# jinbeizame007/pytorch-r2d2-DPG

Hardware: NVIDIA H100
Metric: learner sequence-steps/sec (batch x seq_len) (higher is better)
Workload: dtype bf16x3 (fp32 operands split into bf16 hi+lo, three tensor-core passes, fp32 accumulate: ~16-bit operands)

## Files before the change

include/r2d2_b200.h:

```cpp
#ifndef R2D2_B200_H_
#define R2D2_B200_H_

#include <stddef.h>
#include <stdint.h>

#ifdef __cplusplus
extern "C" {
#endif

#define R2D2_OK 0
#define R2D2_ERR_CUDA (-1)
#define R2D2_ERR_ARG (-2)
#define R2D2_ERR_UNSUPPORTED (-3)
#define R2D2_ERR_STATE (-4)

typedef void* r2d2_stream_t;

int r2d2_version(void);
const char* r2d2_arch(void);
const char* r2d2_last_error(void);
int r2d2_device_sm_count(int* out);

int r2d2_gemm_f32(int layout, int M, int N, int K, const float* A, long long lda, const float* B, long long ldb,
                  const float* A2, long long lda2, const float* B2, long long ldb2, int K2, float* C,
                  long long ldc, const float* bias, const float* Z, long long ldz, int epilogue, int split_k,
                  r2d2_stream_t stream);

typedef struct {
  int obs_size;
  int n_actions;
  int hidden;
  int is_critic;
} r2d2_net_shape;

size_t r2d2_net_param_count(const r2d2_net_shape* shape);
size_t r2d2_net_workspace_floats(const r2d2_net_shape* shape, int T, int B, int repeat);

int r2d2_lstm_net_forward(const r2d2_net_shape* shape, const float* params, const float* obs, const float* act,
                          const float* h0, const float* c0, int T, int B, int repeat, int head_first_row,
                          float* out, float* workspace, r2d2_stream_t stream);

int r2d2_lstm_net_backward(const r2d2_net_shape* shape, const float* params, const float* obs, const float* act,
                           const float* d_out, int T, int B, int repeat, int head_first_row, float* grads,
                           float* d_act, float* workspace, r2d2_stream_t stream);

int r2d2_lstm_scan_forward(const float* gin, const float* whh, const float* h0, const float* c0, float* gates,
                           float* hs, float* cs, float* head_in, int T, int B, int H, int repeat, float* scratch,
                           r2d2_stream_t stream);
int r2d2_lstm_scan_backward(const float* gates, const float* hs, const float* cs, const float* whh,
                            const float* dh_head, int head_first_step, float* dgates, float* dgin, int T, int B,
                            int H, int repeat, float* scratch, r2d2_stream_t stream);

int r2d2_set_gemm_impl(int impl);
int r2d2_get_gemm_impl(void);
int r2d2_set_scan_impl(int impl);
int r2d2_get_scan_impl(void);
int r2d2_scan_status(int* status, r2d2_stream_t stream);

int r2d2_td_priority(const float* q, const float* q_next, const float* rew, const float* term, int L, int B,
                     int A, int burn_in, int n_step, float gamma, float eta, float* target, float* dq,
                     float* td_sq, float* priority, float* critic_loss, r2d2_stream_t stream);
int r2d2_td_priority_weighted(const float* q, const float* q_next, const float* rew, const float* term,
                              const float* is_weight, int L, int B, int A, int burn_in, int n_step, float gamma, float eta,
                              float* target, float* dq, float* td_sq, float* priority, float* critic_loss,
                              r2d2_stream_t stream);

#define R2D2_RESCALE_REFERENCE 0
#define R2D2_RESCALE_INVERTIBLE 1
#define R2D2_PRIORITY_SQUARED 0
#define R2D2_PRIORITY_ABS 1
typedef struct {
  int rescaling;
  float eps;
  int priority_metric;
} r2d2_td_options;
int r2d2_td_priority_ex(const float* q, const float* q_next, const float* rew, const float* term, const float* is_weight,
                        int L, int B, int A, int burn_in, int n_step, float gamma, float eta, float* target, float* dq,
                        float* td_sq, float* priority, float* critic_loss, const r2d2_td_options* options,
                        r2d2_stream_t stream);

int r2d2_nstep_rewards(const float* raw, const int* n_rows, int T, int B, int n_step, float gamma, float* out,
                       r2d2_stream_t stream);
int r2d2_actor_priorities(const float* q, const float* q_next, const float* rew, const float* term, const int* n_rows,
                          int B, int A, int burn_in, int learning, int n_step, float gamma, float eta, int p_max,
                          float* prio, r2d2_stream_t stream);
int r2d2_actor_priorities_ex(const float* q, const float* q_next, const float* rew, const float* term, const int* n_rows,
                             int B, int A, int burn_in, int learning, int n_step, float gamma, float eta, int p_max,
                             float* prio, const r2d2_td_options* options, r2d2_stream_t stream);

size_t r2d2_policy_workspace_floats(const r2d2_net_shape* shape, int N);
int r2d2_policy_step(const r2d2_net_shape* shape, const float* const params[4], const float* obs,
                     const float* state_in, float* state_out, float* mu, int N, float* workspace,
                     r2d2_stream_t stream);

int r2d2_adam_step(float* params, const float* grads, float* exp_avg, float* exp_avg_sq, long long n, int step,
                   float lr, float beta1, float beta2, float eps, float grad_scale, r2d2_stream_t stream);

typedef struct r2d2_replay r2d2_replay_t;

typedef struct {
  int obs_size, n_actions, hidden;
// ... 105 lines not shown
```

pytorch-r2d2-dpg_b200/csrc/api.cu:

```cuda
#include <atomic>
#include <cmath>

#include "common.cuh"
#include "elementwise.cuh"
#include "gemm.cuh"
#include "learner.cuh"
#include "lstm_scan.cuh"
#include "net.cuh"
#include "policy.cuh"
#include "replay.cuh"

namespace r2d2 {
static thread_local std::string g_last_error;
static std::atomic<long long> g_launches{0};
void set_last_error(const std::string& msg) { g_last_error = msg; }
const char* last_error() { return g_last_error.c_str(); }
void count_launch(int n) { g_launches.fetch_add(n, std::memory_order_relaxed); }
long long launch_count() { return g_launches.load(std::memory_order_relaxed); }
int num_sms() {
  static std::atomic<int> cache[64];
  int dev = 0;
  if (cudaGetDevice(&dev) != cudaSuccess || dev < 0 || dev >= 64) return 132;
  int n = cache[dev].load(std::memory_order_relaxed);
  if (n == 0) {
// ... 39 lines not shown

size_t r2d2_net_param_count(const r2d2_net_shape* shape) { return shape ? shape_of(shape).param_count() : 0; }

size_t r2d2_net_workspace_floats(const r2d2_net_shape* shape, int T, int B, int repeat) {
  return shape ? ChainWs::floats(shape_of(shape), T, B, repeat) : 0;
}

int r2d2_lstm_net_forward(const r2d2_net_shape* shape, const float* params, const float* obs, const float* act,
                          const float* h0, const float* c0, int T, int B, int repeat, int head_first_row,
                          float* out, float* workspace, r2d2_stream_t stream) {
  R2D2_REQUIRE(shape && params && obs && workspace, "null");
  R2D2_REQUIRE(T > 0 && B > 0 && repeat >= 1, "shape");
  const NetShape s = shape_of(shape);
  const NetParams P = NetParams::from_flat(const_cast<float*>(params), s);
  const ChainWs ws = ChainWs::carve(workspace, s, T, B, repeat);
  R2D2_TRY(net_forward(s, P, ws, obs, act, h0, c0, T, B, repeat, S(stream)));
  if (out) {
    float* ho = ws.head_out + (size_t)head_first_row * B * s.act;
    R2D2_TRY(net_head_forward(s, P, ws, head_first_row, T, B, repeat, ho, s.act, S(stream)));
    R2D2_CUDA_TRY(cudaMemcpyAsync(out, ho, sizeof(float) * (size_t)(T - head_first_row) * B * s.act,
                                  cudaMemcpyDeviceToDevice, S(stream)));
  }
  return R2D2_OK;
}

int r2d2_lstm_net_backward(const r2d2_net_shape* shape, const float* params, const float* obs, const float* act,
                           const float* d_out, int T, int B, int repeat, int head_first_row, float* grads,
                           float* d_act, float* workspace, r2d2_stream_t stream) {
  R2D2_REQUIRE(shape && params && obs && d_out && workspace, "null");
  const NetShape s = shape_of(shape);
  const NetParams P = NetParams::from_flat(const_cast<float*>(params), s);
  const ChainWs ws = ChainWs::carve(workspace, s, T, B, repeat);
  const long long n = (long long)(T - head_first_row) * B * s.act;
  const float* d_pre = d_out;
  if (!s.critic) {
    R2D2_TRY(mul_dtanh(d_out, ws.head_out + (size_t)head_first_row * B * s.act, ws.d_pre, n, S(stream)));
    d_pre = ws.d_pre;
  }
  NetParams G;
  if (grads) G = NetParams::from_flat(grads, s);
  return net_backward(s, P, grads ? &G : nullptr, ws, obs, act, d_pre, head_first_row, T, B, repeat, d_act, nullptr,
                      S(stream));
}

int r2d2_lstm_scan_forward(const float* gin, const float* whh, const float* h0, const float* c0, float* gates,
                           float* hs, float* cs, float* head_in, int T, int B, int H, int repeat, float* scratch,
                           r2d2_stream_t stream) {
  ScanFwdParams p;
  p.gin = gin; p.whh = whh; p.h0 = h0; p.c0 = c0; p.gates = gates; p.hs = hs; p.cs = cs; p.head_in = head_in;
  p.T = T; p.B = B; p.H = H; p.repeat = repeat; p.scratch = scratch;
  return lstm_scan_forward(p, S(stream));
}

int r2d2_lstm_scan_backward(const float* gates, const float* hs, const float* cs, const float* whh,
                            const float* dh_head, int head_first_step, float* dgates, float* dgin, int T, int B,
                            int H, int repeat, float* scratch, r2d2_stream_t stream) {
  ScanBwdParams p;
  p.gates = gates; p.hs = hs; p.cs = cs; p.whh = whh; p.dh_head = dh_head; p.head_first_step = head_first_step;
  p.dgates = dgates; p.dgin = dgin; p.T = T; p.B = B; p.H = H; p.repeat = repeat; p.scratch = scratch;
  return lstm_scan_backward(p, S(stream));
}

int r2d2_set_gemm_impl(int impl) {
  gemm_set_impl(impl != 0);
  gemm_set_impl_skinny_mma(impl != 2);
  return R2D2_OK;
}
int r2d2_get_gemm_impl(void) { return gemm_get_impl(); }
int r2d2_set_scan_impl(int impl) { lstm_scan_set_impl(impl); return R2D2_OK; }
int r2d2_get_scan_impl(void) { return lstm_scan_get_impl(); }
int r2d2_scan_status(int* status, r2d2_stream_t stream) { return lstm_scan_error_status(status, S(stream)); }

int r2d2_td_priority(const float* q, const float* q_next, const float* rew, const float* term, int L, int B,
                     int A, int burn_in, int n_step, float gamma, float eta, float* target, float* dq,
                     float* td_sq, float* priority, float* critic_loss, r2d2_stream_t stream) {
  TdPriorityParams p;
  p.q = q; p.q_next = q_next; p.rew = rew; p.term = term; p.target = target; p.dq = dq; p.td_sq = td_sq;
  p.priority = priority; p.loss_sum = critic_loss; p.L = L; p.B = B; p.A = A; p.burn_in = burn_in; p.n_step = n_step;
  p.gamma_n = (float)pow((double)gamma, (double)n_step);
  p.eta = eta;
  return td_priority(p, S(stream));
}

int r2d2_td_priority_weighted(const float* q, const float* q_next, const float* rew, const float* term,
                              const float* is_weight, int L, int B, int A, int burn_in, int n_step, float gamma, float eta,
                              float* target, float* dq, float* td_sq, float* priority, float* critic_loss,
                              r2d2_stream_t stream) {
  TdPriorityParams p;
  p.q = q; p.q_next = q_next; p.rew = rew; p.term = term; p.target = target; p.dq = dq; p.td_sq = td_sq;
  p.priority = priority; p.loss_sum = critic_loss; p.L = L; p.B = B; p.A = A; p.burn_in = burn_in; p.n_step = n_step;
  p.gamma_n = (float)pow((double)gamma, (double)n_step);
  p.eta = eta;
  p.is_weight = is_weight;
  return td_priority(p, S(stream));
}

static int td_options_of(const r2d2_td_options* o, TdOptions* out) {
  *out = TdOptions();
  if (o) { out->rescaling = o->rescaling; out->eps = o->eps; out->priority_metric = o->priority_metric; }
  return check_td_options(*out);
}

int r2d2_td_priority_ex(const float* q, const float* q_next, const float* rew, const float* term, const float* is_weight,
                        int L, int B, int A, int burn_in, int n_step, float gamma, float eta, float* target, float* dq,
                        float* td_sq, float* priority, float* critic_loss, const r2d2_td_options* options,
                        r2d2_stream_t stream) {
// ... 243 lines not shown
```

pytorch-r2d2-dpg_b200/csrc/lstm_scan.cu:

```cuda
#include <cooperative_groups.h>
#include <stdlib.h>

#include "gemm.cuh"
#include "lstm_scan.cuh"
#include "elementwise.cuh"
#include "sm90.cuh"

namespace cg = cooperative_groups;

namespace r2d2 {
namespace {

constexpr int SCAN_THREADS = 256;
constexpr int UNITS_PER_CTA = 32;
constexpr int ROWS_PER_CTA = 128;
constexpr int GT_LD = ROWS_PER_CTA + 4;
constexpr int DG_LD = ROWS_PER_CTA + 8;
constexpr unsigned long long kWaitLimitNs = 4000000000ull;

__device__ unsigned g_scan_status = 0;

__device__ __forceinline__ float accurate_sigmoid(float x) { return 1.0f / (1.0f + expf(-x)); }

__device__ __forceinline__ unsigned long long global_ns() {
  unsigned long long t;
  asm volatile("mov.u64 %0, %globaltimer;" : "=l"(t));
  return t;
}

__device__ __forceinline__ void wait_slice(uint64_t* bar, uint32_t parity) {
  if (sm90::mbar_try_wait(bar, parity)) return;
  if (*reinterpret_cast<volatile unsigned*>(&g_scan_status)) return;
  const unsigned long long t0 = global_ns();
  while (!sm90::mbar_try_wait(bar, parity)) {
    if (global_ns() - t0 > kWaitLimitNs) {
      atomicExch(&g_scan_status, 1u);
      return;
    }
  }
}

__device__ __forceinline__ uint32_t slice_parity(int s) { return (uint32_t)((s - 1) >> 1) & 1u; }

template <int H> __host__ __device__ constexpr bool w_hi_in_smem() { return H > 256; }

template <int H, int NB>
struct FwdSmem {
  static constexpr int C = H / 32;
  static constexpr int HROW = UNITS_PER_CTA + 8;
  static constexpr int SLICE = 2 * NB * HROW;
  static constexpr int W_BYTES = w_hi_in_smem<H>() ? (H / 16) * 8 * 32 * 16 : 0;
  static constexpr int HB_ELEMS = 2 * C * SLICE;
  static constexpr int GT_ELEMS = NB * GT_LD;
  static constexpr int HS_ELEMS = SLICE;
  static constexpr int BAR_OFF = W_BYTES + HB_ELEMS * 2 + GT_ELEMS * 4 + HS_ELEMS * 2;
  static constexpr int BYTES = BAR_OFF + 2 * C * 8;
  static_assert((SLICE * 2) % 16 == 0 && BAR_OFF % 16 == 0, "bulk copies need 16-byte granules");
  static_assert(BYTES <= 232448, "forward scan tile does not fit in 227 KB of shared memory");
};

template <int H, int NB>
__global__ void __launch_bounds__(SCAN_THREADS, 1) lstm_scan_fwd_kernel(ScanFwdParams p) {
  constexpr int C = H / 32, KS = H / 16, NT = NB / 8;
  constexpr bool WS = w_hi_in_smem<H>();
  using SM = FwdSmem<H, NB>;
  constexpr int HROW = SM::HROW, SLICE = SM::SLICE;
  cg::cluster_group cluster = cg::this_cluster();
  const int rank = (int)cluster.block_rank();
  const int b0 = (blockIdx.x / C) * NB;
  const int tid = threadIdx.x, lane = tid & 31, w = tid >> 5;
  const int g = lane >> 2, c = lane & 3;
  const int B = p.B, S = p.T * p.repeat;

  extern __shared__ __align__(16) unsigned char smem_raw[];
  uint4* w_hi_s = reinterpret_cast<uint4*>(smem_raw);
  __nv_bfloat16* hb = reinterpret_cast<__nv_bfloat16*>(smem_raw + SM::W_BYTES);
  float* gt = reinterpret_cast<float*>(smem_raw + SM::W_BYTES + SM::HB_ELEMS * 2);
  __nv_bfloat16* hstage = reinterpret_cast<__nv_bfloat16*>(smem_raw + SM::W_BYTES + SM::HB_ELEMS * 2 + SM::GT_ELEMS * 4);
  uint64_t* bar = reinterpret_cast<uint64_t*>(smem_raw + SM::BAR_OFF);

  for (int idx = tid; idx < NB * H; idx += SCAN_THREADS) {
    const int n = idx / H, k = idx % H, b = b0 + n;
    float v = (b < B && p.h0) ? __ldg(p.h0 + (size_t)b * H + k) : 0.f;
    __nv_bfloat16 hi, lo;
    split_bf16(v, hi, lo);
    __nv_bfloat16* row = hb + (0 * C + k / UNITS_PER_CTA) * SLICE + n * HROW + k % UNITS_PER_CTA;
    row[0] = hi;
    row[NB * HROW] = lo;
  }
  const int ug = rank * 32 + lane;
  float cst[NT];
#pragma unroll
  for (int e = 0; e < NT; ++e) {
    const int b = b0 + w + 8 * e;
    cst[e] = 0.f;
    if (b < B) {
      float hv = p.h0 ? __ldg(p.h0 + (size_t)b * H + ug) : 0.f;
      float cv = p.c0 ? __ldg(p.c0 + (size_t)b * H + ug) : 0.f;
      p.hs[(size_t)b * H + ug] = hv;
      p.cs[(size_t)b * H + ug] = cv;
      cst[e] = cv;
    }
  }
  if (tid < 2 * C) {
    sm90::mbar_init(bar + tid, 1);
    sm90::fence_mbar_init_cluster();
    sm90::mbar_arrive_expect_tx(bar + tid, SLICE * 2);
  }

  uint32_t a_hi[WS ? 1 : KS][4], a_lo[KS][4];
  {
    const int gate = w >> 1;
    const int u_lo = (w & 1) * 16 + g;
    const float* w_r0 = p.whh + (size_t)(gate * H + rank * 32 + u_lo) * H;
    const float* w_r1 = w_r0 + (size_t)8 * H;
#pragma unroll
    for (int ks = 0; ks < KS; ++ks) {
      const int k = ks * 16 + 2 * c;
      float2 v0 = __ldg(reinterpret_cast<const float2*>(w_r0 + k));
      float2 v1 = __ldg(reinterpret_cast<const float2*>(w_r1 + k));
      float2 v2 = __ldg(reinterpret_cast<const float2*>(w_r0 + k + 8));
      float2 v3 = __ldg(reinterpret_cast<const float2*>(w_r1 + k + 8));
      uint32_t h[4];
      split_pack2(v0.x, v0.y, h[0], a_lo[ks][0]);
      split_pack2(v1.x, v1.y, h[1], a_lo[ks][1]);
      split_pack2(v2.x, v2.y, h[2], a_lo[ks][2]);
      split_pack2(v3.x, v3.y, h[3], a_lo[ks][3]);
      if constexpr (WS) {
        w_hi_s[(ks * 8 + w) * 32 + lane] = make_uint4(h[0], h[1], h[2], h[3]);
      } else {
#pragma unroll
        for (int f = 0; f < 4; ++f) a_hi[ks][f] = h[f];
      }
    }
  }
  __syncthreads();
  cluster.sync();

  const size_t gstride = (size_t)4 * H;
  for (int s = 0; s < S; ++s) {
    const int cur = s & 1, nxt = cur ^ 1;
    const int t = s / p.repeat;

#pragma unroll
    for (int nt = 0; nt < NT; ++nt)
#pragma unroll
      for (int f = 0; f < 4; ++f) {
        const int n = nt * 8 + 2 * c + (f & 1), r = 16 * w + g + (f >> 1) * 8, b = b0 + n;
        if (b < B) sm90::cp_async_4(gt + n * GT_LD + r, p.gin + ((size_t)t * B + b) * gstride + (r >> 5) * H + rank * 32 + (r & 31));
      }
    sm90::cp_async_commit();

    float acc[NT][4];
#pragma unroll
    for (int nt = 0; nt < NT; ++nt)
#pragma unroll
      for (int e = 0; e < 4; ++e) acc[nt][e] = 0.f;
    const __nv_bfloat16* hb_cur = hb + cur * C * SLICE;
    uint64_t* bar_cur = bar + cur * C;
    const uint32_t parity = slice_parity(s);
#pragma unroll
    for (int ks = 0; ks < KS; ++ks) {
      if ((ks & 1) == 0 && s > 0) wait_slice(bar_cur + ks / 2, parity);
      const __nv_bfloat16* hb_hi = hb_cur + (ks / 2) * SLICE;
      const __nv_bfloat16* hb_lo = hb_hi + NB * HROW;
      uint32_t ah[4];
      if constexpr (WS) {
        const uint4 v = w_hi_s[(ks * 8 + w) * 32 + lane];
        ah[0] = v.x; ah[1] = v.y; ah[2] = v.z; ah[3] = v.w;
      } else {
#pragma unroll
        for (int f = 0; f < 4; ++f) ah[f] = a_hi[ks][f];
      }
#pragma unroll
      for (int nt = 0; nt < NT; ++nt) {
        const int off = (nt * 8 + g) * HROW + (ks & 1) * 16 + 2 * c;
        uint32_t bh[2], bl[2];
        bh[0] = *reinterpret_cast<const uint32_t*>(hb_hi + off);
        bh[1] = *reinterpret_cast<const uint32_t*>(hb_hi + off + 8);
        bl[0] = *reinterpret_cast<const uint32_t*>(hb_lo + off);
        bl[1] = *reinterpret_cast<const uint32_t*>(hb_lo + off + 8);
        mma_bf16_16816(acc[nt], a_lo[ks], bh);
        mma_bf16_16816(acc[nt], ah, bl);
        mma_bf16_16816(acc[nt], ah, bh);
      }
    }
    sm90::cp_async_wait_all();
#pragma unroll
    for (int nt = 0; nt < NT; ++nt) {
      const int n = nt * 8 + 2 * c, r = 16 * w + g;
      gt[n * GT_LD + r] += acc[nt][0];
      gt[(n + 1) * GT_LD + r] += acc[nt][1];
      gt[n * GT_LD + r + 8] += acc[nt][2];
      gt[(n + 1) * GT_LD + r + 8] += acc[nt][3];
    }
    if (w == 0 && lane < C) sm90::bulk_wait_read_all();
    __syncthreads();
    if (s > 0 && tid < C) sm90::mbar_arrive_expect_tx(bar_cur + tid, SLICE * 2);

#pragma unroll
    for (int e = 0; e < NT; ++e) {
      const int n = w + 8 * e, b = b0 + n;
      __nv_bfloat16 hi = __float2bfloat16_rn(0.f), lo = hi;
      if (b < B) {
        const float* gr = gt + n * GT_LD + lane;
        const float ig = accurate_sigmoid(gr[0]);
        const float fg = accurate_sigmoid(gr[32]);
        const float gg = tanhf(gr[64]);
        const float og = accurate_sigmoid(gr[96]);
        const float cn = fg * cst[e] + ig * gg;
        const float hn = og * tanhf(cn);
        cst[e] = cn;
        if (!p.no_save) {
          float* go = p.gates + ((size_t)s * B + b) * gstride + ug;
          go[0] = ig; go[H] = fg; go[2 * H] = gg; go[3 * H] = og;
          p.cs[((size_t)(s + 1) * B + b) * H + ug] = cn;
        }
        p.hs[((size_t)(s + 1) * B + b) * H + ug] = hn;
        if (p.head_in && (s % p.repeat) == p.repeat - 1)
          p.head_in[((size_t)t * B + b) * H + ug] = tanhf(hn);
        split_bf16(hn, hi, lo);
      }
      hstage[(0 * NB + n) * HROW + lane] = hi;
      hstage[(1 * NB + n) * HROW + lane] = lo;
    }
    sm90::fence_proxy_async_smem();
    __syncthreads();

    if (s + 1 < S && w == 0 && lane < C) {
      const uint32_t slot = sm90::smem_u32(hb + (nxt * C + rank) * SLICE);
      const uint32_t slot_bar = sm90::smem_u32(bar + nxt * C + rank);
      sm90::bulk_copy_s2cluster(sm90::map_cluster(slot, lane), sm90::smem_u32(hstage), SLICE * 2,
                                sm90::map_cluster(slot_bar, lane));
      sm90::bulk_commit();
    }
  }
  cluster.sync();
}

template <int H, int NB>
struct BwdSmem {
  static constexpr int C = H / 32;
  static constexpr int DG_ELEMS = 2 * NB * DG_LD;
  static constexpr int PS_LD = NB + 2;
  static constexpr int PS_ELEMS = 2 * C * UNITS_PER_CTA * PS_LD;
  static constexpr int PS_BYTES_PER_SRC = UNITS_PER_CTA * NB * 4;
  static constexpr int MT = (H / 16 + 7) / 8;
  static constexpr int W_BYTES = w_hi_in_smem<H>() ? MT * 8 * 8 * 32 * 16 : 0;
  static constexpr int STAGE_PLANES = 6;
  static constexpr int STAGE_ELEMS = STAGE_PLANES * NB * UNITS_PER_CTA;
  static constexpr int BAR_OFF = W_BYTES + DG_ELEMS * 2 + PS_ELEMS * 4 + STAGE_ELEMS * 4;
  static constexpr int BYTES = BAR_OFF + 2 * C * 8;
  static_assert(BAR_OFF % 8 == 0, "mbarrier alignment");
  static_assert(BYTES <= 232448, "BPTT scan tile does not fit in 227 KB of shared memory");
};

template <int H, int NB>
__global__ void __launch_bounds__(SCAN_THREADS, 1) lstm_scan_bwd_kernel(ScanBwdParams p) {
  constexpr int C = H / 32, NT = NB / 8;
  constexpr int M_TILES = H / 16;
  constexpr int MT = (M_TILES + 7) / 8;
  constexpr int KS = ROWS_PER_CTA / 16;
  constexpr bool WS = w_hi_in_smem<H>();
  using SM = BwdSmem<H, NB>;
  cg::cluster_group cluster = cg::this_cluster();
  const int rank = (int)cluster.block_rank();
  const int b0 = (blockIdx.x / C) * NB;
  const int tid = threadIdx.x, lane = tid & 31, w = tid >> 5;
  const int g = lane >> 2, c = lane & 3;
  const int B = p.B, S = p.T * p.repeat;

  extern __shared__ __align__(16) unsigned char smem_raw[];
  uint4* w_hi_s = reinterpret_cast<uint4*>(smem_raw);
  __nv_bfloat16* dgs = reinterpret_cast<__nv_bfloat16*>(smem_raw + SM::W_BYTES);
  float* ps = reinterpret_cast<float*>(smem_raw + SM::W_BYTES + SM::DG_ELEMS * 2);
  float* stage = ps + SM::PS_ELEMS;
  uint64_t* bar = reinterpret_cast<uint64_t*>(smem_raw + SM::BAR_OFF);
  constexpr int PLANE = NB * UNITS_PER_CTA;
  constexpr size_t gstride = (size_t)4 * H;

  auto head_step = [&](int s) {
    const int rel = s - p.head_first_step;
// ... 307 lines not shown
int set_cluster_attributes(Kern kern, int cluster_size, int smem_bytes) {
  R2D2_CUDA_TRY(cudaFuncSetAttribute(kern, cudaFuncAttributeMaxDynamicSharedMemorySize, smem_bytes));
  if (cluster_size > 8) R2D2_CUDA_TRY(cudaFuncSetAttribute(kern, cudaFuncAttributeNonPortableClusterSizeAllowed, 1));
  return R2D2_OK;
}

cudaLaunchConfig_t cluster_config(int cluster_size, int n_clusters, int smem_bytes, cudaStream_t stream,
                                  cudaLaunchAttribute* attr) {
  cudaLaunchConfig_t cfg = {};
  cfg.gridDim = dim3(cluster_size * n_clusters);
  cfg.blockDim = dim3(SCAN_THREADS);
  cfg.dynamicSmemBytes = smem_bytes;
  cfg.stream = stream;
  attr[0].id = cudaLaunchAttributeClusterDimension;
  attr[0].val.clusterDim.x = cluster_size;
  attr[0].val.clusterDim.y = 1;
  attr[0].val.clusterDim.z = 1;
  cfg.attrs = attr;
  cfg.numAttrs = 1;
  return cfg;
}

template <typename Kern, typename Params>
int launch_cluster(Kern kern, const Params& p, int cluster_size, int n_clusters, int smem_bytes, cudaStream_t stream) {
  R2D2_TRY(set_cluster_attributes(kern, cluster_size, smem_bytes));
  cudaLaunchAttribute attr[1];
  cudaLaunchConfig_t cfg = cluster_config(cluster_size, n_clusters, smem_bytes, stream, attr);
  R2D2_CUDA_TRY(cudaLaunchKernelEx(&cfg, kern, p));
  count_launch();
  return R2D2_OK;
}

template <typename Kern>
int resident_clusters(Kern kern, int cluster_size, int smem_bytes, int* out) {
  R2D2_TRY(set_cluster_attributes(kern, cluster_size, smem_bytes));
  cudaLaunchAttribute attr[1];
  cudaLaunchConfig_t cfg = cluster_config(cluster_size, 1, smem_bytes, nullptr, attr);
  R2D2_CUDA_TRY(cudaOccupancyMaxActiveClusters(out, kern, &cfg));
  return R2D2_OK;
}

template <int H, typename K8, typename K16, typename K32>
int pick_nb(int B, K8 k8, int smem8, K16 k16, int smem16, K32 k32, int smem32, int* nb) {
  int fit = 0;
  R2D2_TRY(resident_clusters(k8, H / 32, smem8, &fit));
  if (ceil_div(B, 8) <= fit) { *nb = 8; return R2D2_OK; }
  R2D2_TRY(resident_clusters(k16, H / 32, smem16, &fit));
  if (ceil_div(B, 16) <= fit || !k32) { *nb = 16; return R2D2_OK; }
  *nb = 32;
  (void)smem32;
  return R2D2_OK;
}

template <int H>
int fwd_dispatch(const ScanFwdParams& p, cudaStream_t stream) {
  constexpr bool WIDE = !w_hi_in_smem<H>();
  constexpr int NB3 = WIDE ? 32 : 16;
  int nb = 0;
  R2D2_TRY(pick_nb<H>(p.B, lstm_scan_fwd_kernel<H, 8>, FwdSmem<H, 8>::BYTES, lstm_scan_fwd_kernel<H, 16>,
                      FwdSmem<H, 16>::BYTES, WIDE ? lstm_scan_fwd_kernel<H, NB3> : nullptr, FwdSmem<H, NB3>::BYTES, &nb));
  if (nb == 8)
    return launch_cluster(lstm_scan_fwd_kernel<H, 8>, p, H / 32, ceil_div(p.B, 8), FwdSmem<H, 8>::BYTES, stream);
  if (nb == 16)
    return launch_cluster(lstm_scan_fwd_kernel<H, 16>, p, H / 32, ceil_div(p.B, 16), FwdSmem<H, 16>::BYTES, stream);
  return launch_cluster(lstm_scan_fwd_kernel<H, NB3>, p, H / 32, ceil_div(p.B, NB3), FwdSmem<H, NB3>::BYTES, stream);
}
template <int H>
int bwd_dispatch(const ScanBwdParams& p, cudaStream_t stream) {
  constexpr bool WIDE = !w_hi_in_smem<H>();
  constexpr int NB3 = WIDE ? 32 : 16;
  int nb = 0;
  R2D2_TRY(pick_nb<H>(p.B, lstm_scan_bwd_kernel<H, 8>, BwdSmem<H, 8>::BYTES, lstm_scan_bwd_kernel<H, 16>,
                      BwdSmem<H, 16>::BYTES, WIDE ? lstm_scan_bwd_kernel<H, NB3> : nullptr, BwdSmem<H, NB3>::BYTES, &nb));
  if (nb == 8)
    return launch_cluster(lstm_scan_bwd_kernel<H, 8>, p, H / 32, ceil_div(p.B, 8), BwdSmem<H, 8>::BYTES, stream);
  if (nb == 16)
    return launch_cluster(lstm_scan_bwd_kernel<H, 16>, p, H / 32, ceil_div(p.B, 16), BwdSmem<H, 16>::BYTES, stream);
  return launch_cluster(lstm_scan_bwd_kernel<H, NB3>, p, H / 32, ceil_div(p.B, NB3), BwdSmem<H, NB3>::BYTES, stream);
}

}

bool lstm_scan_cluster_supported(int H) { return H == 32 || H == 64 || H == 128 || H == 256 || H == 512; }

static int g_scan_impl = -1;
void lstm_scan_set_impl(int impl) { g_scan_impl = impl ? 1 : 0; }
int lstm_scan_get_impl() {
  if (g_scan_impl < 0) {
    const char* e = getenv("R2D2_SCAN_IMPL");
    g_scan_impl = (e && (e[0] == 's' || e[0] == '0')) ? 0 : 1;
  }
  return g_scan_impl;
}
static bool use_cluster_kernels(int H) { return lstm_scan_cluster_supported(H) && lstm_scan_get_impl() == 1; }

int lstm_scan_error_status(int* out, cudaStream_t stream) {
  R2D2_REQUIRE(out, "null");
  unsigned v = 0;
  R2D2_CUDA_TRY(cudaMemcpyFromSymbolAsync(&v, g_scan_status, sizeof(v), 0, cudaMemcpyDeviceToHost, stream));
  R2D2_CUDA_TRY(cudaStreamSynchronize(stream));
  *out = (int)v;
  return R2D2_OK;
}

size_t lstm_scan_fwd_scratch_floats(int B, int H) { return (size_t)B * 4 * H; }
size_t lstm_scan_bwd_scratch_floats(int B, int H) { return (size_t)2 * B * H; }

int lstm_scan_forward(const ScanFwdParams& p, cudaStream_t stream) {
  R2D2_REQUIRE(p.gin && p.whh && p.gates && p.hs && p.cs, "null pointer");
  R2D2_REQUIRE(p.T > 0 && p.B > 0 && p.H > 0 && p.repeat >= 1, "shape");
  R2D2_REQUIRE(p.repeat == 1 || p.gates != p.gin, "gates must not alias gin when repeat > 1");
  if (use_cluster_kernels(p.H)) {
    switch (p.H) {
      case 32: return fwd_dispatch<32>(p, stream);
      case 64: return fwd_dispatch<64>(p, stream);
      case 128: return fwd_dispatch<128>(p, stream);
      case 256: return fwd_dispatch<256>(p, stream);
      case 512: return fwd_dispatch<512>(p, stream);
// ... 29 lines not shown
```

pytorch-r2d2-dpg_b200/csrc/lstm_scan.cuh:

```cuda
#pragma once
#include "common.cuh"

namespace r2d2 {

struct ScanFwdParams {
  const float* gin = nullptr;
  const float* whh = nullptr;
  const float* h0 = nullptr;
  const float* c0 = nullptr;
  float* gates = nullptr;
  float* hs = nullptr;
  float* cs = nullptr;
  float* head_in = nullptr;
  int T = 0, B = 0, H = 0, repeat = 1;
  float* scratch = nullptr;
  int no_save = 0;
};

struct ScanBwdParams {
  const float* gates = nullptr;
  const float* hs = nullptr;
  const float* cs = nullptr;
  const float* whh = nullptr;
  const float* dh_head = nullptr;
  int head_first_step = 0;
  float* dgates = nullptr;
  float* dgin = nullptr;
  int T = 0, B = 0, H = 0, repeat = 1;
  float* scratch = nullptr;
  float* dbias = nullptr;
  float* dbias2 = nullptr;
};

bool lstm_scan_cluster_supported(int H);
int lstm_scan_forward(const ScanFwdParams& p, cudaStream_t stream);
int lstm_scan_backward(const ScanBwdParams& p, cudaStream_t stream);
size_t lstm_scan_fwd_scratch_floats(int B, int H);
size_t lstm_scan_bwd_scratch_floats(int B, int H);

void lstm_scan_set_impl(int impl);
int lstm_scan_get_impl();
int lstm_scan_error_status(int* out, cudaStream_t stream);

}
```

pytorch-r2d2-dpg_b200/csrc/sm90.cuh:

```cuda
#pragma once
#include <cuda_runtime.h>
#include <stdint.h>

namespace r2d2 {
namespace sm90 {

__device__ __forceinline__ uint32_t smem_u32(const void* p) { return (uint32_t)__cvta_generic_to_shared(p); }

__device__ __forceinline__ uint64_t make_smem_desc(uint32_t smem_addr, uint32_t lbo_bytes, uint32_t sbo_bytes) {
  uint64_t d = 0;
  d |= (uint64_t)((smem_addr >> 4) & 0x3FFF);
  d |= (uint64_t)((lbo_bytes >> 4) & 0x3FFF) << 16;
  d |= (uint64_t)((sbo_bytes >> 4) & 0x3FFF) << 32;
  return d;
}

__device__ __forceinline__ void wgmma_fence() { asm volatile("wgmma.fence.sync.aligned;" ::: "memory"); }
__device__ __forceinline__ void wgmma_commit() { asm volatile("wgmma.commit_group.sync.aligned;" ::: "memory"); }
template <int N>
__device__ __forceinline__ void wgmma_wait() { asm volatile("wgmma.wait_group.sync.aligned %0;" ::"n"(N) : "memory"); }
__device__ __forceinline__ void fence_regs(float (&d)[64]) {
#pragma unroll
  for (int i = 0; i < 64; ++i) asm volatile("" : "+f"(d[i])::"memory");
}
// ... 36 lines not shown
      "}\n"
      : "=r"(pred));
  return pred != 0;
}

__device__ __forceinline__ void mbar_init(uint64_t* bar, uint32_t count) {
  asm volatile("mbarrier.init.shared::cta.b64 [%0], %1;" ::"r"(smem_u32(bar)), "r"(count) : "memory");
}
__device__ __forceinline__ void mbar_arrive(uint64_t* bar) {
  asm volatile("mbarrier.arrive.shared::cta.b64 _, [%0];" ::"r"(smem_u32(bar)) : "memory");
}
__device__ __forceinline__ void mbar_arrive_expect_tx(uint64_t* bar, uint32_t tx_bytes) {
  asm volatile("mbarrier.arrive.expect_tx.shared::cta.b64 _, [%0], %1;" ::"r"(smem_u32(bar)), "r"(tx_bytes) : "memory");
}
__device__ __forceinline__ bool mbar_try_wait(uint64_t* bar, uint32_t parity) {
  uint32_t ok;
  asm volatile(
      "{\n\t"
      ".reg .pred p;\n\t"
      "mbarrier.try_wait.parity.shared::cta.b64 p, [%1], %2;\n\t"
      "selp.u32 %0, 1, 0, p;\n\t"
      "}\n"
      : "=r"(ok)
      : "r"(smem_u32(bar)), "r"(parity)
      : "memory");
  return ok != 0;
}

__device__ __forceinline__ void bulk_copy_g2s(uint32_t dst_smem_addr, const void* src_global, uint32_t bytes, uint32_t mbar_smem_addr) {
  asm volatile("cp.async.bulk.shared::cluster.global.mbarrier::complete_tx::bytes [%0], [%1], %2, [%3];" ::"r"(dst_smem_addr),
               "l"(src_global), "r"(bytes), "r"(mbar_smem_addr)
               : "memory");
}

__device__ __forceinline__ void cp_async_4(float* smem_dst, const float* gsrc) {
  asm volatile("cp.async.ca.shared.global [%0], [%1], 4;" ::"r"((uint32_t)__cvta_generic_to_shared(smem_dst)), "l"(gsrc) : "memory");
}
__device__ __forceinline__ void cp_async_commit() { asm volatile("cp.async.commit_group;" ::: "memory"); }
__device__ __forceinline__ void cp_async_wait_all() { asm volatile("cp.async.wait_group 0;" ::: "memory"); }

__device__ __forceinline__ void fence_mbar_init_cluster() { asm volatile("fence.mbarrier_init.release.cluster;" ::: "memory"); }
__device__ __forceinline__ void fence_proxy_async_smem() { asm volatile("fence.proxy.async.shared::cta;" ::: "memory"); }
__device__ __forceinline__ uint32_t map_cluster(uint32_t smem_addr, uint32_t rank) {
  uint32_t r;
  asm volatile("mapa.shared::cluster.u32 %0, %1, %2;" : "=r"(r) : "r"(smem_addr), "r"(rank));
  return r;
}
__device__ __forceinline__ void bulk_copy_s2cluster(uint32_t dst_cluster_addr, uint32_t src_smem_addr, uint32_t bytes,
                                                    uint32_t mbar_cluster_addr) {
  asm volatile("cp.async.bulk.shared::cluster.shared::cta.mbarrier::complete_tx::bytes [%0], [%1], %2, [%3];"
               ::"r"(dst_cluster_addr), "r"(src_smem_addr), "r"(bytes), "r"(mbar_cluster_addr)
               : "memory");
}
__device__ __forceinline__ void bulk_commit() { asm volatile("cp.async.bulk.commit_group;" ::: "memory"); }
__device__ __forceinline__ void bulk_wait_read_all() { asm volatile("cp.async.bulk.wait_group.read 0;" ::: "memory"); }
__device__ __forceinline__ void st_async_f2(uint32_t dst_cluster_addr, float x, float y, uint32_t mbar_cluster_addr) {
  asm volatile("st.async.shared::cluster.mbarrier::complete_tx::bytes.v2.f32 [%0], {%1, %2}, [%3];"
               ::"r"(dst_cluster_addr), "f"(x), "f"(y), "r"(mbar_cluster_addr)
               : "memory");
}

}
}
```

pytorch-r2d2-dpg_b200/r2d2_b200/native.py:

```python
from __future__ import annotations

import ctypes
import os
from ctypes import POINTER, Structure, byref, c_char_p, c_double, c_float, c_int, c_longlong, c_size_t, c_void_p

import numpy as np
import torch

_HERE = os.path.dirname(os.path.abspath(__file__))
LIB_PATH = os.environ.get("R2D2_B200_LIB") or os.path.join(os.path.dirname(_HERE), "libr2d2_b200.so")

GEMM_NT, GEMM_NN, GEMM_TN = 0, 1, 2
EPI_NONE, EPI_TANH, EPI_MUL_DTANH, EPI_ADD_Z = 0, 1, 2, 3


class NativeError(RuntimeError):
    pass


class NetShape(Structure):
    _fields_ = [("obs_size", c_int), ("n_actions", c_int), ("hidden", c_int), ("is_critic", c_int)]


class ReplayConfig(Structure):
    _fields_ = [("obs_size", c_int), ("n_actions", c_int), ("hidden", c_int), ("burn_in", c_int),
                ("learning", c_int), ("n_step", c_int), ("capacity_rows", c_longlong),
                ("max_sequences", c_longlong)]


class ReplayStats(Structure):
    _fields_ = [("n_episodes", c_longlong), ("n_rows_used", c_longlong), ("sequence_counter", c_longlong),
                ("capacity_rows", c_longlong), ("tree_levels", c_longlong), ("tree_nodes", c_longlong),
                ("last_row_start", c_longlong), ("total_priority", c_double)]


class LearnerConfig(Structure):
    _fields_ = [("obs_size", c_int), ("n_actions", c_int), ("hidden", c_int), ("batch", c_int),
                ("burn_in", c_int), ("learning", c_int), ("n_step", c_int), ("gamma", c_float),
                ("actor_lr", c_float), ("critic_lr", c_float), ("eta", c_float),
                ("target_update_interval", c_int),
                ("actor_params", c_void_p), ("critic_params", c_void_p), ("target_actor_params", c_void_p),
                ("target_critic_params", c_void_p), ("actor_grads", c_void_p), ("critic_grads", c_void_p),
                ("actor_exp_avg", c_void_p), ("actor_exp_avg_sq", c_void_p), ("critic_exp_avg", c_void_p),
                ("critic_exp_avg_sq", c_void_p)]


class TdOptions(Structure):
    _fields_ = [("rescaling", c_int), ("eps", c_float), ("priority_metric", c_int)]


class PeerLayout(Structure):
    _fields_ = [(k, c_size_t) for k in ("bytes", "off_critic_grads", "off_actor_grads", "off_critic_sums",
                                        "off_actor_sums")]


class LearnerBuffers(Structure):
    _fields_ = [(k, c_void_p) for k in ("obs", "act", "rew", "term", "states", "leaf_idx", "uniforms",
                                        "q_value", "target_q_value", "td_sq", "priority", "losses")]


SIGNATURES = {
    "r2d2_version": (c_int, []),
    "r2d2_arch": (c_char_p, []),
    "r2d2_last_error": (c_char_p, []),
    "r2d2_device_sm_count": (c_int, [POINTER(c_int)]),
    "r2d2_gemm_f32": (c_int, [c_int, c_int, c_int, c_int, c_void_p, c_longlong, c_void_p, c_longlong, c_void_p,
                              c_longlong, c_void_p, c_longlong, c_int, c_void_p, c_longlong, c_void_p, c_void_p,
                              c_longlong, c_int, c_int, c_void_p]),
    "r2d2_net_param_count": (c_size_t, [POINTER(NetShape)]),
    "r2d2_net_workspace_floats": (c_size_t, [POINTER(NetShape), c_int, c_int, c_int]),
    "r2d2_lstm_net_forward": (c_int, [POINTER(NetShape), c_void_p, c_void_p, c_void_p, c_void_p, c_void_p, c_int,
                                      c_int, c_int, c_int, c_void_p, c_void_p, c_void_p]),
    "r2d2_lstm_net_backward": (c_int, [POINTER(NetShape), c_void_p, c_void_p, c_void_p, c_void_p, c_int, c_int,
                                       c_int, c_int, c_void_p, c_void_p, c_void_p, c_void_p]),
    "r2d2_lstm_scan_forward": (c_int, [c_void_p, c_void_p, c_void_p, c_void_p, c_void_p, c_void_p, c_void_p, c_void_p,
                                       c_int, c_int, c_int, c_int, c_void_p, c_void_p]),
    "r2d2_lstm_scan_backward": (c_int, [c_void_p, c_void_p, c_void_p, c_void_p, c_void_p, c_int, c_void_p, c_void_p,
                                        c_int, c_int, c_int, c_int, c_void_p, c_void_p]),
    "r2d2_set_gemm_impl": (c_int, [c_int]),
    "r2d2_get_gemm_impl": (c_int, []),
    "r2d2_set_scan_impl": (c_int, [c_int]),
    "r2d2_get_scan_impl": (c_int, []),
    "r2d2_scan_status": (c_int, [POINTER(c_int), c_void_p]),
    "r2d2_td_priority": (c_int, [c_void_p, c_void_p, c_void_p, c_void_p, c_int, c_int, c_int, c_int, c_int, c_float,
                                 c_float, c_void_p, c_void_p, c_void_p, c_void_p, c_void_p, c_void_p]),
    "r2d2_td_priority_weighted": (c_int, [c_void_p, c_void_p, c_void_p, c_void_p, c_void_p, c_int, c_int, c_int, c_int,
                                          c_int, c_float, c_float, c_void_p, c_void_p, c_void_p, c_void_p, c_void_p,
                                          c_void_p]),
    "r2d2_td_priority_ex": (c_int, [c_void_p, c_void_p, c_void_p, c_void_p, c_void_p, c_int, c_int, c_int, c_int, c_int,
                                    c_float, c_float, c_void_p, c_void_p, c_void_p, c_void_p, c_void_p,
                                    POINTER(TdOptions), c_void_p]),
    "r2d2_nstep_rewards": (c_int, [c_void_p, c_void_p, c_int, c_int, c_int, c_float, c_void_p, c_void_p]),
    "r2d2_actor_priorities": (c_int, [c_void_p, c_void_p, c_void_p, c_void_p, c_void_p, c_int, c_int, c_int, c_int, c_int,
                                      c_float, c_float, c_int, c_void_p, c_void_p]),
    "r2d2_actor_priorities_ex": (c_int, [c_void_p, c_void_p, c_void_p, c_void_p, c_void_p, c_int, c_int, c_int, c_int,
                                         c_int, c_float, c_float, c_int, c_void_p, POINTER(TdOptions), c_void_p]),
    "r2d2_policy_workspace_floats": (c_size_t, [POINTER(NetShape), c_int]),
    "r2d2_policy_step": (c_int, [POINTER(NetShape), POINTER(c_void_p), c_void_p, c_void_p, c_void_p, c_void_p, c_int,
                                 c_void_p, c_void_p]),
    "r2d2_adam_step": (c_int, [c_void_p, c_void_p, c_void_p, c_void_p, c_longlong, c_int, c_float, c_float, c_float,
                               c_float, c_float, c_void_p]),
    "r2d2_replay_create": (c_int, [POINTER(c_void_p), POINTER(ReplayConfig)]),
    "r2d2_replay_destroy": (c_int, [c_void_p]),
    "r2d2_replay_set_priority_exponent": (c_int, [c_void_p, c_float]),
    "r2d2_replay_add_episodes": (c_int, [c_void_p, c_int, c_void_p, c_void_p, c_void_p, c_void_p, c_void_p, c_void_p, c_void_p,
                                         c_void_p, c_void_p, c_void_p, c_void_p, c_void_p]),
    "r2d2_replay_add_episode": (c_int, [c_void_p, c_void_p, c_void_p, c_void_p, c_void_p, c_void_p, c_int, c_int,
                                        c_void_p, c_int, c_void_p]),
    "r2d2_replay_sample": (c_int, [c_void_p, c_void_p, c_int, c_void_p, c_void_p, c_void_p, c_void_p, c_void_p,
                                   c_void_p, c_void_p]),
    "r2d2_replay_sample_weighted": (c_int, [c_void_p, c_void_p, c_int, c_float, c_void_p, c_void_p, c_void_p, c_void_p,
                                            c_void_p, c_void_p, c_void_p, c_void_p]),
    "r2d2_replay_gather": (c_int, [c_void_p, c_void_p, c_int, c_void_p, c_void_p, c_void_p, c_void_p, c_void_p, c_void_p]),
    "r2d2_replay_update_priorities": (c_int, [c_void_p, c_void_p, c_void_p, c_int, c_void_p]),
    "r2d2_replay_stats": (c_int, [c_void_p, POINTER(ReplayStats), c_void_p]),
    "r2d2_replay_decode": (c_int, [c_void_p, c_void_p, c_int, c_void_p, c_void_p]),
    "r2d2_replay_tree_level": (c_int, [c_void_p, c_int, POINTER(c_void_p), POINTER(c_longlong)]),
    "r2d2_learner_create": (c_int, [POINTER(c_void_p), POINTER(LearnerConfig)]),
    "r2d2_learner_destroy": (c_int, [c_void_p]),
    "r2d2_learner_buffers_get": (c_int, [c_void_p, POINTER(LearnerBuffers)]),
    "r2d2_learner_critic_phase": (c_int, [c_void_p, c_void_p]),
    "r2d2_learner_actor_forward": (c_int, [c_void_p, c_void_p]),
    "r2d2_learner_actor_phase": (c_int, [c_void_p, c_float, c_void_p]),
    "r2d2_learner_finish_phase": (c_int, [c_void_p, c_float, c_void_p]),
    "r2d2_learner_step_count": (c_int, [c_void_p]),
    "r2d2_learner_set_step_count": (c_int, [c_void_p, c_int]),
    "r2d2_learner_set_overlap_actor_inputs": (c_int, [c_void_p, c_int]),
    "r2d2_learner_buffers_get_slot": (c_int, [c_void_p, c_int, POINTER(LearnerBuffers)]),
    "r2d2_learner_select_batch": (c_int, [c_void_p, c_int]),
# ... 77 lines not shown
```

Before: 1.118 million.

## Single-buffer forward scan h-slices with slot-free barriers and split batch launches

When the double-buffered forward LSTM scan tile does not fit in shared memory, it now uses one h-buffer. The CTA's own slice doubles as the staging area, and new per-slot 'slot_free' mbarriers, signalled remotely by each peer CTA, gate when the next bulk copy may overwrite a slot. The dispatcher can also split the batch into a wave-sized NB=32 launch plus an NB=16 remainder launch, using new b_begin/b_end range parameters. The aim is to let larger batch tiles fit and stay resident, at the cost of an extra cross-CTA handshake per step and a second kernel launch. It also adds a forward_ex API with a no_save flag and a launch-count query.

New measurement: 1.138 million (median of 6 runs). 1.9% higher.

```diff
diff --git a/include/r2d2_b200.h b/include/r2d2_b200.h
--- a/include/r2d2_b200.h
+++ b/include/r2d2_b200.h
@@ -47,6 +47,10 @@
 int r2d2_lstm_scan_forward(const float* gin, const float* whh, const float* h0, const float* c0, float* gates,
                            float* hs, float* cs, float* head_in, int T, int B, int H, int repeat, float* scratch,
                            r2d2_stream_t stream);
+int r2d2_lstm_scan_forward_ex(const float* gin, const float* whh, const float* h0, const float* c0, float* gates,
+                              float* hs, float* cs, float* head_in, int T, int B, int H, int repeat, int no_save,
+                              float* scratch, r2d2_stream_t stream);
+long long r2d2_launch_count(void);
 int r2d2_lstm_scan_backward(const float* gates, const float* hs, const float* cs, const float* whh,
                             const float* dh_head, int head_first_step, float* dgates, float* dgin, int T, int B,
                             int H, int repeat, float* scratch, r2d2_stream_t stream);
diff --git a/pytorch-r2d2-dpg_b200/csrc/api.cu b/pytorch-r2d2-dpg_b200/csrc/api.cu
--- a/pytorch-r2d2-dpg_b200/csrc/api.cu
+++ b/pytorch-r2d2-dpg_b200/csrc/api.cu
@@ -115,6 +115,17 @@
   return lstm_scan_forward(p, S(stream));
 }
 
+int r2d2_lstm_scan_forward_ex(const float* gin, const float* whh, const float* h0, const float* c0, float* gates,
+                              float* hs, float* cs, float* head_in, int T, int B, int H, int repeat, int no_save,
+                              float* scratch, r2d2_stream_t stream) {
+  ScanFwdParams p;
+  p.gin = gin; p.whh = whh; p.h0 = h0; p.c0 = c0; p.gates = gates; p.hs = hs; p.cs = cs; p.head_in = head_in;
+  p.T = T; p.B = B; p.H = H; p.repeat = repeat; p.scratch = scratch; p.no_save = no_save ? 1 : 0;
+  return lstm_scan_forward(p, S(stream));
+}
+
+long long r2d2_launch_count(void) { return launch_count(); }
+
 int r2d2_lstm_scan_backward(const float* gates, const float* hs, const float* cs, const float* whh,
                             const float* dh_head, int head_first_step, float* dgates, float* dgin, int T, int B,
                             int H, int repeat, float* scratch, r2d2_stream_t stream) {
diff --git a/pytorch-r2d2-dpg_b200/csrc/lstm_scan.cu b/pytorch-r2d2-dpg_b200/csrc/lstm_scan.cu
--- a/pytorch-r2d2-dpg_b200/csrc/lstm_scan.cu
+++ b/pytorch-r2d2-dpg_b200/csrc/lstm_scan.cu
@@ -50,11 +50,13 @@
   static constexpr int HROW = UNITS_PER_CTA + 8;
   static constexpr int SLICE = 2 * NB * HROW;
   static constexpr int W_BYTES = w_hi_in_smem<H>() ? (H / 16) * 8 * 32 * 16 : 0;
-  static constexpr int HB_ELEMS = 2 * C * SLICE;
   static constexpr int GT_ELEMS = NB * GT_LD;
-  static constexpr int HS_ELEMS = SLICE;
+  static constexpr bool SINGLE = W_BYTES + (2 * C + 1) * SLICE * 2 + GT_ELEMS * 4 + 2 * C * 8 > 232448;
+  static constexpr int NBUF = SINGLE ? 1 : 2;
+  static constexpr int HB_ELEMS = NBUF * C * SLICE;
+  static constexpr int HS_ELEMS = SINGLE ? 0 : SLICE;
   static constexpr int BAR_OFF = W_BYTES + HB_ELEMS * 2 + GT_ELEMS * 4 + HS_ELEMS * 2;
-  static constexpr int BYTES = BAR_OFF + 2 * C * 8;
+  static constexpr int BYTES = BAR_OFF + (NBUF + SINGLE) * C * 8;
   static_assert((SLICE * 2) % 16 == 0 && BAR_OFF % 16 == 0, "bulk copies need 16-byte granules");
   static_assert(BYTES <= 232448, "forward scan tile does not fit in 227 KB of shared memory");
 };
@@ -64,24 +66,29 @@
   constexpr int C = H / 32, KS = H / 16, NT = NB / 8;
   constexpr bool WS = w_hi_in_smem<H>();
   using SM = FwdSmem<H, NB>;
+  constexpr bool SB = SM::SINGLE;
   constexpr int HROW = SM::HROW, SLICE = SM::SLICE;
   cg::cluster_group cluster = cg::this_cluster();
   const int rank = (int)cluster.block_rank();
-  const int b0 = (blockIdx.x / C) * NB;
+  constexpr bool RANGE = WS;
+  const int b0 = (RANGE ? p.b_begin : 0) + (blockIdx.x / C) * NB;
   const int tid = threadIdx.x, lane = tid & 31, w = tid >> 5;
   const int g = lane >> 2, c = lane & 3;
-  const int B = p.B, S = p.T * p.repeat;
+  const int B = p.B, b_end = RANGE ? p.b_end : p.B, S = p.T * p.repeat;
 
   extern __shared__ __align__(16) unsigned char smem_raw[];
   uint4* w_hi_s = reinterpret_cast<uint4*>(smem_raw);
   __nv_bfloat16* hb = reinterpret_cast<__nv_bfloat16*>(smem_raw + SM::W_BYTES);
   float* gt = reinterpret_cast<float*>(smem_raw + SM::W_BYTES + SM::HB_ELEMS * 2);
-  __nv_bfloat16* hstage = reinterpret_cast<__nv_bfloat16*>(smem_raw + SM::W_BYTES + SM::HB_ELEMS * 2 + SM::GT_ELEMS * 4);
+  __nv_bfloat16* hstage = SB ? hb + rank * SLICE
+                             : reinterpret_cast<__nv_bfloat16*>(smem_raw + SM::W_BYTES + SM::HB_ELEMS * 2 + SM::GT_ELEMS * 4);
   uint64_t* bar = reinterpret_cast<uint64_t*>(smem_raw + SM::BAR_OFF);
+  uint64_t* slot_free = bar + SM::NBUF * C;
+  const auto peer = [&](int r) { return !SB || r != rank; };
 
   for (int idx = tid; idx < NB * H; idx += SCAN_THREADS) {
     const int n = idx / H, k = idx % H, b = b0 + n;
-    float v = (b < B && p.h0) ? __ldg(p.h0 + (size_t)b * H + k) : 0.f;
+    float v = (b < b_end && p.h0) ? __ldg(p.h0 + (size_t)b * H + k) : 0.f;
     __nv_bfloat16 hi, lo;
     split_bf16(v, hi, lo);
     __nv_bfloat16* row = hb + (0 * C + k / UNITS_PER_CTA) * SLICE + n * HROW + k % UNITS_PER_CTA;
@@ -94,7 +101,7 @@
   for (int e = 0; e < NT; ++e) {
     const int b = b0 + w + 8 * e;
     cst[e] = 0.f;
-    if (b < B) {
+    if (b < b_end) {
       float hv = p.h0 ? __ldg(p.h0 + (size_t)b * H + ug) : 0.f;
       float cv = p.c0 ? __ldg(p.c0 + (size_t)b * H + ug) : 0.f;
       p.hs[(size_t)b * H + ug] = hv;
@@ -102,10 +109,16 @@
       cst[e] = cv;
     }
   }
-  if (tid < 2 * C) {
+  if (tid < SM::NBUF * C && peer(tid % C)) {
     sm90::mbar_init(bar + tid, 1);
     sm90::fence_mbar_init_cluster();
     sm90::mbar_arrive_expect_tx(bar + tid, SLICE * 2);
+  }
+  if constexpr (SB) {
+    if (tid >= 32 && tid < 32 + C) {
+      sm90::mbar_init(slot_free + tid - 32, 1);
+      sm90::fence_mbar_init_cluster();
+    }
   }
 
   uint32_t a_hi[WS ? 1 : KS][4], a_lo[KS][4];
@@ -139,7 +152,7 @@
 
   const size_t gstride = (size_t)4 * H;
   for (int s = 0; s < S; ++s) {
-    const int cur = s & 1, nxt = cur ^ 1;
+    const int cur = SB ? 0 : s & 1, nxt = SB ? 0 : cur ^ 1;
     const int t = s / p.repeat;
 
 #pragma unroll
@@ -147,7 +160,7 @@
 #pragma unroll
       for (int f = 0; f < 4; ++f) {
         const int n = nt * 8 + 2 * c + (f & 1), r = 16 * w + g + (f >> 1) * 8, b = b0 + n;
-        if (b < B) sm90::cp_async_4(gt + n * GT_LD + r, p.gin + ((size_t)t * B + b) * gstride + (r >> 5) * H + rank * 32 + (r & 31));
+        if (b < b_end) sm90::cp_async_4(gt + n * GT_LD + r, p.gin + ((size_t)t * B + b) * gstride + (r >> 5) * H + rank * 32 + (r & 31));
       }
     sm90::cp_async_commit();
 
@@ -158,10 +171,10 @@
       for (int e = 0; e < 4; ++e) acc[nt][e] = 0.f;
     const __nv_bfloat16* hb_cur = hb + cur * C * SLICE;
     uint64_t* bar_cur = bar + cur * C;
-    const uint32_t parity = slice_parity(s);
+    const uint32_t parity = SB ? (uint32_t)(s - 1) & 1u : slice_parity(s);
 #pragma unroll
     for (int ks = 0; ks < KS; ++ks) {
-      if ((ks & 1) == 0 && s > 0) wait_slice(bar_cur + ks / 2, parity);
+      if ((ks & 1) == 0 && s > 0 && peer(ks / 2)) wait_slice(bar_cur + ks / 2, parity);
       const __nv_bfloat16* hb_hi = hb_cur + (ks / 2) * SLICE;
       const __nv_bfloat16* hb_lo = hb_hi + NB * HROW;
       uint32_t ah[4];
@@ -196,13 +209,17 @@
     }
     if (w == 0 && lane < C) sm90::bulk_wait_read_all();
     __syncthreads();
-    if (s > 0 && tid < C) sm90::mbar_arrive_expect_tx(bar_cur + tid, SLICE * 2);
+    if (s > 0 && tid < C && peer(tid)) sm90::mbar_arrive_expect_tx(bar_cur + tid, SLICE * 2);
+    if constexpr (SB) {
+      if (s + 1 < S && tid < C && tid != rank)
+        sm90::mbar_arrive_remote(sm90::map_cluster(sm90::smem_u32(slot_free + rank), tid));
+    }
 
 #pragma unroll
     for (int e = 0; e < NT; ++e) {
       const int n = w + 8 * e, b = b0 + n;
       __nv_bfloat16 hi = __float2bfloat16_rn(0.f), lo = hi;
-      if (b < B) {
+      if (b < b_end) {
         const float* gr = gt + n * GT_LD + lane;
         const float ig = accurate_sigmoid(gr[0]);
         const float fg = accurate_sigmoid(gr[32]);
@@ -227,7 +244,8 @@
     sm90::fence_proxy_async_smem();
     __syncthreads();
 
-    if (s + 1 < S && w == 0 && lane < C) {
+    if (s + 1 < S && w == 0 && lane < C && peer(lane)) {
+      if constexpr (SB) wait_slice(slot_free + lane, (uint32_t)s & 1u);
       const uint32_t slot = sm90::smem_u32(hb + (nxt * C + rank) * SLICE);
       const uint32_t slot_bar = sm90::smem_u32(bar + nxt * C + rank);
       sm90::bulk_copy_s2cluster(sm90::map_cluster(slot, lane), sm90::smem_u32(hstage), SLICE * 2,
@@ -641,18 +659,37 @@
   return R2D2_OK;
 }
 
+template <int H, int NB>
+int fwd_launch(ScanFwdParams p, int b_begin, int b_end, cudaStream_t stream) {
+  p.b_begin = b_begin;
+  p.b_end = b_end;
+  return launch_cluster(lstm_scan_fwd_kernel<H, NB>, p, H / 32, ceil_div(b_end - b_begin, NB), FwdSmem<H, NB>::BYTES,
+                        stream);
+}
+
 template <int H>
 int fwd_dispatch(const ScanFwdParams& p, cudaStream_t stream) {
-  constexpr bool WIDE = !w_hi_in_smem<H>();
-  constexpr int NB3 = WIDE ? 32 : 16;
-  int nb = 0;
-  R2D2_TRY(pick_nb<H>(p.B, lstm_scan_fwd_kernel<H, 8>, FwdSmem<H, 8>::BYTES, lstm_scan_fwd_kernel<H, 16>,
-                      FwdSmem<H, 16>::BYTES, WIDE ? lstm_scan_fwd_kernel<H, NB3> : nullptr, FwdSmem<H, NB3>::BYTES, &nb));
-  if (nb == 8)
-    return launch_cluster(lstm_scan_fwd_kernel<H, 8>, p, H / 32, ceil_div(p.B, 8), FwdSmem<H, 8>::BYTES, stream);
-  if (nb == 16)
-    return launch_cluster(lstm_scan_fwd_kernel<H, 16>, p, H / 32, ceil_div(p.B, 16), FwdSmem<H, 16>::BYTES, stream);
-  return launch_cluster(lstm_scan_fwd_kernel<H, NB3>, p, H / 32, ceil_div(p.B, NB3), FwdSmem<H, NB3>::BYTES, stream);
+  const int B = p.B;
+  if constexpr (!FwdSmem<H, 32>::SINGLE) {
+    int nb = 0;
+    R2D2_TRY(pick_nb<H>(B, lstm_scan_fwd_kernel<H, 8>, FwdSmem<H, 8>::BYTES, lstm_scan_fwd_kernel<H, 16>,
+                        FwdSmem<H, 16>::BYTES, lstm_scan_fwd_kernel<H, 32>, FwdSmem<H, 32>::BYTES, &nb));
+    if (nb == 8) return fwd_launch<H, 8>(p, 0, B, stream);
+    if (nb == 16) return fwd_launch<H, 16>(p, 0, B, stream);
+    return fwd_launch<H, 32>(p, 0, B, stream);
+  } else {
+    int fit8 = 0, fit16 = 0, fit32 = 0;
+    R2D2_TRY(resident_clusters(lstm_scan_fwd_kernel<H, 8>, H / 32, FwdSmem<H, 8>::BYTES, &fit8));
+    if (ceil_div(B, 8) <= fit8) return fwd_launch<H, 8>(p, 0, B, stream);
+    R2D2_TRY(resident_clusters(lstm_scan_fwd_kernel<H, 16>, H / 32, FwdSmem<H, 16>::BYTES, &fit16));
+    if (ceil_div(B, 16) <= fit16) return fwd_launch<H, 16>(p, 0, B, stream);
+    R2D2_TRY(resident_clusters(lstm_scan_fwd_kernel<H, 32>, H / 32, FwdSmem<H, 32>::BYTES, &fit32));
+    const int wave = 32 * fit32;
+    const int split = wave > 0 ? B / wave * wave : 0;
+    if (split == 0 || split == B || ceil_div(B - split, 16) > fit16) return fwd_launch<H, 32>(p, 0, B, stream);
+    R2D2_TRY((fwd_launch<H, 32>(p, 0, split, stream)));
+    return fwd_launch<H, 16>(p, split, B, stream);
+  }
 }
 template <int H>
 int bwd_dispatch(const ScanBwdParams& p, cudaStream_t stream) {
diff --git a/pytorch-r2d2-dpg_b200/csrc/lstm_scan.cuh b/pytorch-r2d2-dpg_b200/csrc/lstm_scan.cuh
--- a/pytorch-r2d2-dpg_b200/csrc/lstm_scan.cuh
+++ b/pytorch-r2d2-dpg_b200/csrc/lstm_scan.cuh
@@ -15,6 +15,7 @@
   int T = 0, B = 0, H = 0, repeat = 1;
   float* scratch = nullptr;
   int no_save = 0;
+  int b_begin = 0, b_end = 0;
 };
 
 struct ScanBwdParams {
diff --git a/pytorch-r2d2-dpg_b200/csrc/sm90.cuh b/pytorch-r2d2-dpg_b200/csrc/sm90.cuh
--- a/pytorch-r2d2-dpg_b200/csrc/sm90.cuh
+++ b/pytorch-r2d2-dpg_b200/csrc/sm90.cuh
@@ -112,6 +112,9 @@
                ::"r"(dst_cluster_addr), "r"(src_smem_addr), "r"(bytes), "r"(mbar_cluster_addr)
                : "memory");
 }
+__device__ __forceinline__ void mbar_arrive_remote(uint32_t mbar_cluster_addr) {
+  asm volatile("mbarrier.arrive.shared::cluster.b64 _, [%0];" ::"r"(mbar_cluster_addr) : "memory");
+}
 __device__ __forceinline__ void bulk_commit() { asm volatile("cp.async.bulk.commit_group;" ::: "memory"); }
 __device__ __forceinline__ void bulk_wait_read_all() { asm volatile("cp.async.bulk.wait_group.read 0;" ::: "memory"); }
 __device__ __forceinline__ void st_async_f2(uint32_t dst_cluster_addr, float x, float y, uint32_t mbar_cluster_addr) {
diff --git a/pytorch-r2d2-dpg_b200/r2d2_b200/native.py b/pytorch-r2d2-dpg_b200/r2d2_b200/native.py
--- a/pytorch-r2d2-dpg_b200/r2d2_b200/native.py
+++ b/pytorch-r2d2-dpg_b200/r2d2_b200/native.py
@@ -75,6 +75,9 @@
                                        c_int, c_int, c_void_p, c_void_p, c_void_p, c_void_p]),
     "r2d2_lstm_scan_forward": (c_int, [c_void_p, c_void_p, c_void_p, c_void_p, c_void_p, c_void_p, c_void_p, c_void_p,
                                        c_int, c_int, c_int, c_int, c_void_p, c_void_p]),
+    "r2d2_lstm_scan_forward_ex": (c_int, [c_void_p, c_void_p, c_void_p, c_void_p, c_void_p, c_void_p, c_void_p,
+                                          c_void_p, c_int, c_int, c_int, c_int, c_int, c_void_p, c_void_p]),
+    "r2d2_launch_count": (c_longlong, []),
     "r2d2_lstm_scan_backward": (c_int, [c_void_p, c_void_p, c_void_p, c_void_p, c_void_p, c_int, c_void_p, c_void_p,
                                         c_int, c_int, c_int, c_int, c_void_p, c_void_p]),
     "r2d2_set_gemm_impl": (c_int, [c_int]),
```
